# ghostop14/gr-clenabled

Measured on AMD Instinct MI355X. Metric: MSamples/sec (complex-float) through clFFT 4096 fwd + window + shift, higher is better.
Workload: dtype f32; 1 GPU; BASELINE configs[1]: forward clFFT 4096-pt complex, blackman window + fftshift, 16384 frames/step/GPU device-resident (1 GiB in+out); fft_size=4096, parallelism=replica-per-gpu x1

## Files before the change

### gr-clenabled_amd/csrc/fft.hip

```cpp
#include <cmath>
#include <cstdlib>
#include <vector>

#include "common.h"
#include "fft_core.hpp"
#include "fft_mr.h"

using namespace fftc;
#ifndef MI355_FFT_WPE
#define MI355_FFT_WPE 3
#endif

namespace {

typedef float f2v __attribute__((ext_vector_type(2)));

template <int N, bool REAL, class G>
__device__ __forceinline__ void load_group(c32 (&v)[16], const void *__restrict__ in, int grp, int tid, int nframes, int in_xor)
{
    using P = Plan<N>;
    constexpr int TH = G::TH, PTS = G::PTS, F = G::F, R0 = P::radix(0), B0 = N / R0;
    const int frames_left = nframes - grp * F;
    if constexpr (N <= 64) {
        (void)in_xor;
#pragma unroll
        for (int k = 0; k < 16; k++) {
            const unsigned e = (unsigned)(tid + TH * k);
            const bool ok = (int)(e / N) < frames_left;
            if constexpr (REAL) {
                const float x = __builtin_nontemporal_load((const float *)in + (size_t)grp * PTS + (ok ? e : 0u));
                v[k] = mk(ok ? x : 0.f, 0.f);
            } else {
                const f2v x = __builtin_nontemporal_load((const f2v *)in + (size_t)grp * PTS + (ok ? e : 0u));
                v[k] = ok ? mk(x.x, x.y) : mk(0.f, 0.f);
            }
        }
        return;
    }
#pragma unroll
    for (int q = 0; q < 16 / R0; q++) {
        const int g = tid + TH * q, fr = g / B0;
        const bool ok = (F == 1) || fr < frames_left;
        const unsigned off = (unsigned)((ok ? fr * N : 0) + (g % B0));
#pragma unroll
        for (int r = 0; r < R0; r++) {
            const unsigned e = off + (unsigned)((r * B0) ^ in_xor);
            if constexpr (REAL) {
                const float x = __builtin_nontemporal_load((const float *)in + (size_t)grp * PTS + e);
                v[q * R0 + r] = mk(ok ? x : 0.f, 0.f);
            } else {
                const f2v x = __builtin_nontemporal_load((const f2v *)in + (size_t)grp * PTS + e);
                v[q * R0 + r] = ok ? mk(x.x, x.y) : mk(0.f, 0.f);
            }
        }
    }
}

template <int N, int SIGN, bool REAL, int PF, class G>
__global__ __launch_bounds__(G::TH, (N <= 4096 ? (PF == 2 ? 2 : MI355_FFT_WPE) : 1)) void k_fft(const void *__restrict__ in, c32 *__restrict__ out,
                                                                 const float *__restrict__ window,
                                                                 const c32 *__restrict__ twtab, int nframes, int ngroups,
                                                                 int shift)
{
    using P = Plan<N>;
    constexpr int TH = G::TH, PTS = G::PTS, F = G::F, NP = P::NP;
    constexpr bool SMALL = N <= 64;
    constexpr int PAD = (N / P::radix(0)) > 1 ? (N / P::radix(0)) : 1;
    constexpr int LDS_SLOTS = SMALL ? PTS + (PTS / N) * PAD : (NP > 1 ? PTS : 1);
    __shared__ c32 lds[LDS_SLOTS];
    const int tid0 = threadIdx.x;
    const int in_xor = (SIGN > 0 && shift) ? (N >> 1) : 0;
    const int out_xor = (SIGN < 0 && shift) ? (N >> 1) : 0;

    TwRegs<N> tw;
    load_twiddles<N, false, G>(tw, tid0, twtab);
    constexpr int R0 = P::radix(0), B0 = N / R0;
    float win[16];
    if constexpr (SMALL) {
        win[0] = window[tid0 % N];
    } else {
#pragma unroll
        for (int q = 0; q < 16 / R0; q++) {
            const int j = (tid0 + TH * q) % B0;
#pragma unroll
            for (int r = 0; r < R0; r++) win[q * R0 + r] = window[j + ((r * B0) ^ in_xor)];
        }
    }

    auto body = [&](c32 (&cur)[16], int grp, int tid) {
        const int frames_left = nframes - grp * F;
        c32 v[16];
        if constexpr (SMALL) {
            const float wv = win[0];
            const int pos = (tid % N) ^ in_xor, fr0 = tid / N;
#pragma unroll
            for (int k = 0; k < 16; k++) {
                const int fr = fr0 + k * (TH / N);
                lds[fr * (N + PAD) + pos] = scale(cur[k], wv);
            }
            __syncthreads();
#pragma unroll
            for (int q = 0; q < 16 / R0; q++) {
                const int g = tid + TH * q, base = (g / B0) * (N + PAD) + (g % B0);
#pragma unroll
                for (int r = 0; r < R0; r++) v[q * R0 + r] = lds[base + r * B0];
            }
            __syncthreads();
        } else {
#pragma unroll
            for (int s = 0; s < 16; s++) v[s] = scale(cur[s], win[s]);
        }
        transform_regs<N, SIGN, false, G>(v, tw, lds, tid);
        if constexpr (SMALL) {
            constexpr int RL = P::radix(NP - 1), BL = N / RL;
            if constexpr (NP > 1) __syncthreads();
#pragma unroll
            for (int q = 0; q < 16 / RL; q++) {
                const int g = tid + TH * q, base = (g / BL) * (N + PAD) + (g % BL);
#pragma unroll
                for (int s = 0; s < RL; s++) lds[base + ((orev<RL>(s) * BL) ^ out_xor)] = v[q * RL + s];
            }
            __syncthreads();
            f2v *__restrict__ out_g = (f2v *)out + (size_t)grp * PTS;
            const int pos = tid % N, fr0 = tid / N;
#pragma unroll
            for (int k = 0; k < 16; k++) {
                const int fr = fr0 + k * (TH / N);
                if (fr < frames_left) {
                    const c32 z = lds[fr * (N + PAD) + pos];
                    f2v o;
                    o.x = z.x;
                    o.y = z.y;
                    __builtin_nontemporal_store(o, out_g + tid + TH * k);
                }
            }
        } else {
            constexpr int RL = P::radix(NP - 1), BL = N / RL;
            f2v *__restrict__ out_g = (f2v *)out + (size_t)grp * PTS;
#pragma unroll
            for (int q = 0; q < 16 / RL; q++) {
                const int g = tid + TH * q, fr = g / BL;
                const unsigned off = (unsigned)(fr * N + (g % BL));
                if ((F == 1) || fr < frames_left) {
#pragma unroll
                    for (int s = 0; s < RL; s++) {
                        f2v o;
                        o.x = v[q * RL + s].x;
                        o.y = v[q * RL + s].y;
                        __builtin_nontemporal_store(o, out_g + off + (unsigned)((orev<RL>(s) * BL) ^ out_xor));
                    }
                }
            }
        }
        if constexpr (NP > 1 || SMALL) __syncthreads();
    };
    const int stride = gridDim.x;
    if constexpr (PF == 2) {
        c32 b0[16], b1[16], b2[16];
        int grp = blockIdx.x;
        if (grp < ngroups) load_group<N, REAL, G>(b0, in, grp, tid0, nframes, in_xor);
        if (grp + stride < ngroups) load_group<N, REAL, G>(b1, in, grp + stride, tid0, nframes, in_xor);
#define MI355_FFT_STEP(CUR, FREE)                                                                   \
        {                                                                                           \
            if (grp >= ngroups) break;                                                              \
            int tid = tid0;                                                                         \
            asm volatile("" : "+v"(tid));                                                           \
            if (grp + 2 * stride < ngroups) load_group<N, REAL, G>(FREE, in, grp + 2 * stride, tid, nframes, in_xor); \
            __builtin_amdgcn_sched_barrier(0);                                                      \
            body(CUR, grp, tid);                                                                    \
            grp += stride;                                                                          \
        }
        for (;;) {
            MI355_FFT_STEP(b0, b2)
            MI355_FFT_STEP(b1, b0)
            MI355_FFT_STEP(b2, b1)
        }
#undef MI355_FFT_STEP
    } else {
        c32 cur[16];
        if ((int)blockIdx.x < ngroups) load_group<N, REAL, G>(cur, in, blockIdx.x, tid0, nframes, in_xor);
        for (int grp = blockIdx.x; grp < ngroups; grp += stride) {
            int tid = tid0;
            asm volatile("" : "+v"(tid));
            c32 nxt[16];
            if constexpr (PF == 1) {
                const int gnext = grp + stride;
                if (gnext < ngroups) load_group<N, REAL, G>(nxt, in, gnext, tid, nframes, in_xor);
                __builtin_amdgcn_sched_barrier(0);
            } else if (grp != (int)blockIdx.x) {
                load_group<N, REAL, G>(cur, in, grp, tid, nframes, in_xor);
            }
            body(cur, grp, tid);
            if constexpr (PF == 1) {
#pragma unroll
                for (int s = 0; s < 16; s++) cur[s] = nxt[s];
            }
        }
    }
}

typedef float f4v __attribute__((ext_vector_type(4)));
__host__ __device__ constexpr float cos128(int m)
{
    constexpr float t[128] = {1.0f, 0.99879545f, 0.99518472f, 0.989176512f, 0.980785251f, 0.970031261f, 0.956940353f, 0.941544056f, 0.923879504f, 0.903989315f, 0.881921291f, 0.857728601f, 0.831469595f, 0.803207517f, 0.773010433f, 0.740951121f, 0.707106769f, 0.671558976f, 0.634393275f, 0.59569931f, 0.555570245f, 0.514102757f, 0.471396744f, 0.427555084f, 0.382683426f, 0.336889863f, 0.290284663f, 0.242980182f, 0.195090324f, 0.146730468f, 0.0980171412f, 0.0490676761f, 0.0f, -0.0490676761f, -0.0980171412f, -0.146730468f, -0.195090324f, -0.242980182f, -0.290284663f, -0.336889863f, -0.382683426f, -0.427555084f, -0.471396744f, -0.514102757f, -0.555570245f, -0.59569931f, -0.634393275f, -0.671558976f, -0.707106769f, -0.740951121f, -0.773010433f, -0.803207517f, -0.831469595f, -0.857728601f, -0.881921291f, -0.903989315f, -0.923879504f, -0.941544056f, -0.956940353f, -0.970031261f, -0.980785251f, -0.989176512f, -0.99518472f, -0.99879545f, -1.0f, -0.99879545f, -0.99518472f, -0.989176512f, -0.980785251f, -0.970031261f, -0.956940353f, -0.941544056f, -0.923879504f, -0.903989315f, -0.881921291f, -0.857728601f, -0.831469595f, -0.803207517f, -0.773010433f, -0.740951121f, -0.707106769f, -0.671558976f, -0.634393275f, -0.59569931f, -0.555570245f, -0.514102757f, -0.471396744f, -0.427555084f, -0.382683426f, -0.336889863f, -0.290284663f, -0.242980182f, -0.195090324f, -0.146730468f, -0.0980171412f, -0.0490676761f, 0.0f, 0.0490676761f, 0.0980171412f, 0.146730468f, 0.195090324f, 0.242980182f, 0.290284663f, 0.336889863f, 0.382683426f, 0.427555084f, 0.471396744f, 0.514102757f, 0.555570245f, 0.59569931f, 0.634393275f, 0.671558976f, 0.707106769f, 0.740951121f, 0.773010433f, 0.803207517f, 0.831469595f, 0.857728601f, 0.881921291f, 0.903989315f, 0.923879504f, 0.941544056f, 0.956940353f, 0.970031261f, 0.980785251f, 0.989176512f, 0.99518472f, 0.99879545f};
    return t[m & 127];
}
__host__ __device__ constexpr float circ_cos(int m, int circ) { return cos128(m * (128 / circ)); }
__host__ __device__ constexpr float circ_sin(int m, int circ) { return cos128(m * (128 / circ) - 32); }
static_assert(circ_cos(0, 128) == 1.0f && circ_cos(32, 128) == 0.0f && circ_cos(16, 128) == 0.707106781f && circ_sin(32, 128) == 1.0f &&
                  circ_sin(8, 64) == 0.707106781f && circ_cos(16, 32) == -1.0f, "twiddle table");

template <int SIGN, bool REAL>
__global__ __launch_bounds__(512, 2) void k_fft_32k(const void *__restrict__ in, c32 *__restrict__ out, const float *__restrict__ window,
                                                    const c32 *__restrict__ twN, int nframes, int shift)
{
    constexpr int N = 32768, NS = 4096, S = 8, H = 4, BL = 256;
    using G = Geo<NS>;
    __shared__ c32 sm[4 * NS];
    const int set = threadIdx.x >> 8, tid0 = threadIdx.x & 255;
    c32 *lds = sm + set * 2 * NS;
    const int in_xor = (SIGN > 0 && shift) ? 8 : 0;
    const int m_xor = (SIGN < 0 && shift) ? (S / 2) : 0;

#ifndef PFR32K
#define PFR32K 0
#endif
    constexpr int PFW = REAL ? 2 : 4, PFR = REAL ? 2 * PFR32K : PFR32K;
    f4v pf[PFR > 0 ? PFR : 1][PFW];
    auto fetch = [&](int frame, int j, int tid, f4v (&t)[PFW]) {
        const unsigned n = (unsigned)(tid + (((8 * set + j) ^ in_xor) * BL));
        const f4v *p = (const f4v *)in + (size_t)frame * (REAL ? N / 4 : N / 2) + (size_t)n * PFW;
#pragma unroll
        for (int k = 0; k < PFW; k++) t[k] = p[k];
    };
    if ((int)blockIdx.x < nframes) {
#pragma unroll
        for (int j = 0; j < PFR; j++) fetch(blockIdx.x, j, tid0, pf[j]);
    }
    for (int frame = blockIdx.x; frame < nframes; frame += gridDim.x) {
        int tid = tid0;
        asm volatile("" : "+v"(tid));
        c32 v[H][16];
        auto load_frame = [&](auto set_tag) {
            constexpr int SET = decltype(set_tag)::value, OTHER = 1 - SET;
#pragma unroll
            for (int j = 0; j < 8; j++) {
                const int r = 8 * SET + j;
                const unsigned n = (unsigned)(tid + ((r ^ in_xor) * BL));
                const f4v wa = *((const f4v *)window + (size_t)n * 2), wb = *((const f4v *)window + (size_t)n * 2 + 1);
                const float w[8] = {wa.x, wa.y, wa.z, wa.w, wb.x, wb.y, wb.z, wb.w};
                f4v t[PFW];
                if (j < PFR) {
#pragma unroll
                    for (int k = 0; k < PFW; k++) t[k] = pf[j][k];
                } else {
                    fetch(frame, j, tid, t);
                }
                c32 x[S];
                if constexpr (REAL) {
#pragma unroll
// ... 470 lines not shown
        for (int i = 0; i < 32; i++) {
            const int e = tid + TH * i, col = e & 15, row = e >> 4;
            c32 x = pf[i];
            if constexpr (!PASS_B) {
                const float w = window[(size_t)(row ^ row_xor) * ld + c0 + col];
                x = mk(x.x * w, x.y * w);
            }
            tile_lds[col * CS + row] = x;
        }
        __syncthreads();
        c32 va[16], vb[16];
        constexpr int R0 = PL::radix(0), B0 = NR / R0;
#pragma unroll
        for (int q = 0; q < 16 / R0; q++) {
            const int g = tid + TH * q, fr = g / B0, j = g % B0;
#pragma unroll
            for (int r = 0; r < R0; r++) {
                va[q * R0 + r] = tile_lds[fr * CS + j + r * B0];
                vb[q * R0 + r] = tile_lds[(fr + 8) * CS + j + r * B0];
            }
        }
        __syncthreads();
        if (item + gridDim.x < nitems) fetch(item + gridDim.x, pf, tid);
        transform_regs2<NR, SIGN, REV, G>(va, vb, tw, tile_lds, tile_lds + 8 * NR, tid);
        constexpr int NP = PL::NP, RL = PL::radix(NP - 1), BL = NR / RL;
        if constexpr (!PASS_B) {
            static_assert(RL == 16, "reversed plan: the last pass is radix 16");
            const int fr = tid / BL, j = tid % BL;
#pragma unroll
            for (int h = 0; h < 2; h++) {
                const int n2 = c0 + fr + 8 * h;
                const c32 base = twN[(int)(((long long)n2 * j) & nmask)], g1 = twN[(int)(((long long)n2 * BL) & nmask)];
                const c32 g2 = cmul(g1, g1), g4 = cmul(g2, g2), g8 = cmul(g4, g4);
                c32 gp[16];
                gp[0] = base;
                gp[1] = cmul(base, g1);
                gp[2] = cmul(base, g2);
                gp[3] = cmul(gp[2], g1);
                gp[4] = cmul(base, g4);
                gp[5] = cmul(gp[4], g1);
                gp[6] = cmul(gp[4], g2);
                gp[7] = cmul(gp[6], g1);
#pragma unroll
                for (int m = 0; m < 8; m++) gp[8 + m] = cmul(gp[m], g8);
                f2v *__restrict__ o = (f2v *)out + (size_t)frame * frame_elems + (size_t)n2 * NR + j;
#pragma unroll
                for (int t = 0; t < 16; t++) {
                    const c32 z = cmul(h ? vb[t] : va[t], gp[orev<16>(t)]);
                    f2v zz;
                    zz.x = z.x;
                    zz.y = z.y;
                    o[orev<16>(t) * BL] = zz;
                }
            }
            __syncthreads();
        } else {
            __syncthreads();
#pragma unroll
            for (int q = 0; q < 16 / RL; q++) {
                const int g = tid + TH * q, fr = g / BL, j = g % BL;
#pragma unroll
                for (int t = 0; t < RL; t++) {
                    tile_lds[fr * CS + j + orev<RL>(t) * BL] = va[q * RL + t];
                    tile_lds[(fr + 8) * CS + j + orev<RL>(t) * BL] = vb[q * RL + t];
                }
            }
            __syncthreads();
#pragma unroll
            for (int i = 0; i < 32; i++) {
                const int e = tid + TH * i, col = e & 15, row = e >> 4;
                const c32 z = tile_lds[col * CS + row];
                f2v zz;
                zz.x = z.x;
                zz.y = z.y;
                __builtin_nontemporal_store(zz, (f2v *)out + (size_t)frame * frame_elems + (size_t)(row ^ row_xor) * ld + c0 + col);
            }
            __syncthreads();
        }
    }
}

template <int N, class G>
int launch_g(mi355_ctx *ctx, int sign, const void *in, void *out, const float *window, const void *tw, int nframes, int shift,
             int real_in, hipStream_t st)
{
    constexpr int F = G::F, TH = G::TH, WAVES = TH / 64;
    int ngroups = (nframes + F - 1) / F;
    int cus = ctx->num_cus > 0 ? ctx->num_cus : 256;
    int pf = getenv("MI355_FFT_PREFETCH") ? atoi(getenv("MI355_FFT_PREFETCH")) : -1;
    const bool persistent2 = N <= 4096 && WAVES == 4 && ngroups >= cus * 2 * 8;
    if (pf < 0) pf = persistent2 ? 1 : 0;
    int grid = (N <= 4096) ? mi355_balanced_grid(ctx, ngroups, 32 / WAVES, 64 / WAVES, 0.015) : mi355_balanced_grid(ctx, ngroups, 1, 1);
    if (pf == 1 && persistent2) grid = cus * 2;
    if (const char *e = getenv("MI355_FFT_WG_PER_CU")) {
        if (atoi(e) > 0) grid = ngroups < cus * atoi(e) ? ngroups : cus * atoi(e);
    }
#define LAUNCH_FFT(SG, RL)                                                                                              \
    do {                                                                                                                     \
        if (pf == 2)                                                                                                         \
            hipLaunchKernelGGL((k_fft<N, SG, RL, 2, G>), dim3(grid), dim3(TH), 0, st, in, (c32 *)out, window, (const c32 *)tw, \
                               nframes, ngroups, shift);                                                                     \
        else if (pf == 1)                                                                                                    \
            hipLaunchKernelGGL((k_fft<N, SG, RL, 1, G>), dim3(grid), dim3(TH), 0, st, in, (c32 *)out, window, (const c32 *)tw, \
                               nframes, ngroups, shift);                                                                     \
        else                                                                                                                 \
            hipLaunchKernelGGL((k_fft<N, SG, RL, 0, G>), dim3(grid), dim3(TH), 0, st, in, (c32 *)out, window,                \
                               (const c32 *)tw, nframes, ngroups, shift);                                                    \
    } while (0)
    if (sign < 0) { if (real_in) LAUNCH_FFT(-1, true); else LAUNCH_FFT(-1, false); }
    else          { if (real_in) LAUNCH_FFT(1, true);  else LAUNCH_FFT(1, false); }
#undef LAUNCH_FFT
    MI355_HIP(hipGetLastError());
    return MI355_OK;
}

template <int N>
int launch_n(mi355_ctx *ctx, int sign, const void *in, void *out, const float *window, const void *tw, int nframes, int shift,
             int real_in, hipStream_t st)
{
    if constexpr (N >= 16 && N <= 1024) {
        static const bool wave = getenv("MI355_FFT_WAVE_GEO") ? atoi(getenv("MI355_FFT_WAVE_GEO")) != 0 : false;
        if (wave) return launch_g<N, GeoW<N>>(ctx, sign, in, out, window, tw, nframes, shift, real_in, st);
    }
    if constexpr (N == 32768) return launch_s<N>(ctx, sign, in, out, window, tw, nframes, shift, real_in, st);
    else if constexpr (N == 8192 || N == 16384) {
        static const bool whole = getenv("MI355_FFT_WHOLE_FRAME") ? atoi(getenv("MI355_FFT_WHOLE_FRAME")) != 0 : false;
        if (!whole) return launch_s<N>(ctx, sign, in, out, window, tw, nframes, shift, real_in, st);
    }
    if constexpr (N != 32768) return launch_g<N, Geo<N>>(ctx, sign, in, out, window, tw, nframes, shift, real_in, st);
}

int launch_fft(mi355_ctx *ctx, int n, int sign, const void *in, void *out, const float *window, const void *tw, int nframes,
               int shift, int real_in, hipStream_t st)
{
    switch (n) {
#define CASE_N(NN) case NN: return launch_n<NN>(ctx, sign, in, out, window, tw, nframes, shift, real_in, st)
        CASE_N(2); CASE_N(4); CASE_N(8); CASE_N(16); CASE_N(32); CASE_N(64); CASE_N(128); CASE_N(256); CASE_N(512);
        CASE_N(1024); CASE_N(2048); CASE_N(4096); CASE_N(8192); CASE_N(16384); CASE_N(32768);
#undef CASE_N
    }
    mi355_set_error("fft size %d unsupported (power of two, 2..32768)", n);
    return MI355_ERR_UNSUPPORTED;
}

}

struct mi355_fft {
    mi355_ctx *ctx;
    int n, sign, dtype, nstreams, shift;
    float *d_window;
    void *d_tw;
    HostPipe pipe;
    MrPlan mr;
    MrTilePlan mrt;
    int m = 0;
    void *d_pre = nullptr, *d_post = nullptr, *d_bspec = nullptr;
    void *d_twm_f = nullptr, *d_twm_i = nullptr;
    float *d_ones = nullptr;
    mi355_fft *sub_f = nullptr, *sub_i = nullptr;
    void *d_wa = nullptr, *d_wb = nullptr;
    size_t cap_frames = 0;
    bool two_kernel = false;
    int tile_n1 = 0, tile_n2 = 0;
    std::mutex ws_lock;
    hipEvent_t ws_done = nullptr;
    bool ws_used = false;
};

namespace {

__global__ __launch_bounds__(256) void k_blu_pre(const void *__restrict__ in, c32 *__restrict__ A, const c32 *__restrict__ pre,
                                                 const int *__restrict__ src, int N, int M, long long total, int real_in)
{
    for (long long e = (long long)blockIdx.x * 256 + threadIdx.x; e < total; e += (long long)gridDim.x * 256) {
        const long long f = e / M;
        const int m = (int)(e - f * M);
        c32 v = mk(0.f, 0.f);
        if (m < N) {
            const int i = src[m];
            const c32 x = real_in ? mk(((const float *)in)[f * N + i], 0.f) : ((const c32 *)in)[f * N + i];
            v = cmul(x, pre[m]);
        }
        A[e] = v;
    }
}

__global__ __launch_bounds__(256) void k_blu_mul(c32 *__restrict__ B, const c32 *__restrict__ bspec, int M, long long total)
{
    for (long long e = (long long)blockIdx.x * 256 + threadIdx.x; e < total; e += (long long)gridDim.x * 256)
        B[e] = cmul(B[e], bspec[e & (M - 1)]);
}

__global__ __launch_bounds__(256) void k_blu_post(const c32 *__restrict__ A, c32 *__restrict__ out, const c32 *__restrict__ post,
                                                  int N, int M, long long total, int lo)
{
    for (long long e = (long long)blockIdx.x * 256 + threadIdx.x; e < total; e += (long long)gridDim.x * 256) {
        const long long f = e / N;
        const int p = (int)(e - f * N);
        const int k = lo ? (p < N - lo ? p + lo : p - (N - lo)) : p;
        out[e] = cmul(A[f * M + k], post[k]);
    }
}

template <int M, bool REAL>
__global__ __launch_bounds__(Geo<M>::TH, Geo<M>::WPE) void k_chirpz(const void *__restrict__ in, c32 *__restrict__ out,
                                                                   const c32 *__restrict__ pre, const int *__restrict__ src,
                                                                   const c32 *__restrict__ post, const c32 *__restrict__ bspec,
                                                                   const c32 *__restrict__ tw_fwd, const c32 *__restrict__ tw_inv,
                                                                   int N, int nframes, int ngroups, int lo)
{
    using G = Geo<M>;
    using PF = Plan<M, false>;
    using PI = Plan<M, true>;
    constexpr int TH = G::TH, F = G::F, NP = PF::NP;
    constexpr int RL = PF::radix(NP - 1), BL = M / RL;
    static_assert(PI::radix(0) == RL, "inverse plan must start with the forward plan's last radix");
    extern __shared__ __attribute__((aligned(16))) c32 chirp_lds[];
    c32 *lds = chirp_lds;
    const int tid0 = threadIdx.x;
    constexpr bool SHARE = (PF::L % 4) == 0;
    TwRegs<M> twf, twi;
    load_twiddles<M, false, G>(twf, tid0, tw_fwd);
    if constexpr (!SHARE) load_twiddles<M, true, G>(twi, tid0, tw_inv);
    c32 Breg[16];
#pragma unroll
    for (int q = 0; q < 16 / RL; q++) {
        const int j = (tid0 + TH * q) % BL;
#pragma unroll
        for (int t = 0; t < RL; t++) Breg[q * RL + t] = bspec[j + orev<RL>(t) * BL];
    }
    for (int grp = blockIdx.x; grp < ngroups; grp += gridDim.x) {
        int tid = tid0;
        asm volatile("" : "+v"(tid));
        const int frames_left = nframes - grp * F;
        const size_t fbase = (size_t)grp * F;
        c32 v[16];
        constexpr int R0 = PF::radix(0), B0 = M / R0;
#pragma unroll
        for (int q = 0; q < 16 / R0; q++) {
            const int g = tid + TH * q, fr = g / B0, j = g % B0;
#pragma unroll
            for (int r = 0; r < R0; r++) {
                const int m = j + r * B0;
                const bool ok = m < N && fr < frames_left;
                c32 x = mk(0.f, 0.f);
                if (ok) {
                    const int i = src[m];
                    if constexpr (REAL) x = mk(((const float *)in)[(fbase + fr) * N + i], 0.f);
// ... 255 lines not shown
            }
            {
                const long long total = (long long)nf * 1048576;
                long long blocks = (total + 255) / 256;
                if (blocks > (long long)cus * 16) blocks = (long long)cus * 16;
                const int mx = (h->sign < 0 && h->shift) ? S3 / 2 : 0;
#define COMB2G(SS) do { if (h->sign < 0) COMB2(SS, -1, 1, (const c32 *)h->d_wa, dst, (const c32 *)h->d_tw, total, 1048576, (long long)N, 1048576LL, 0LL, 0LL, 1, N - 1, mx); \
                        else             COMB2(SS, 1, 1, (const c32 *)h->d_wa, dst, (const c32 *)h->d_tw, total, 1048576, (long long)N, 1048576LL, 0LL, 0LL, 1, N - 1, mx); } while (0)
                if (S3 == 2) COMB2G(2); else if (S3 == 4) COMB2G(4); else if (S3 == 8) COMB2G(8); else COMB2G(16);
#undef COMB2G
            }
            MI355_HIP(hipGetLastError());
            continue;
        }
        if (three_pass) {
            const int S2 = S / 16;
            {
                const long long total = (long long)nf * 4096;
                long long blocks = (total + 255) / 256;
                if (blocks > (long long)cus * 16 / S2 + 1) blocks = (long long)cus * 16 / S2 + 1;
                if (h->sign < 0) COMB2(16, -1, S2, (const c32 *)h->d_wa, (c32 *)h->d_wb, (const c32 *)h->d_tw, total, 4096, (long long)N, (long long)S2 * 4096, 4096LL, 65536LL, S2, N - 1, 0);
                else             COMB2(16, 1, S2, (const c32 *)h->d_wa, (c32 *)h->d_wb, (const c32 *)h->d_tw, total, 4096, (long long)N, (long long)S2 * 4096, 4096LL, 65536LL, S2, N - 1, 0);
            }
            {
                const long long total = (long long)nf * 65536;
                long long blocks = (total + 255) / 256;
                if (blocks > (long long)cus * 16) blocks = (long long)cus * 16;
                const int mx = (h->sign < 0 && h->shift) ? S2 / 2 : 0;
#define COMB2F(SS) do { if (h->sign < 0) COMB2(SS, -1, 1, (const c32 *)h->d_wb, dst, (const c32 *)h->d_tw, total, 65536, (long long)N, 65536LL, 0LL, 0LL, 1, N - 1, mx); \
                        else             COMB2(SS, 1, 1, (const c32 *)h->d_wb, dst, (const c32 *)h->d_tw, total, 65536, (long long)N, 65536LL, 0LL, 0LL, 1, N - 1, mx); } while (0)
                if (S2 == 2) COMB2F(2); else if (S2 == 4) COMB2F(4); else if (S2 == 8) COMB2F(8); else COMB2F(16);
#undef COMB2F
            }
            MI355_HIP(hipGetLastError());
            continue;
        }
#undef COMB2
        const long long total = (long long)nf * 4096;
        long long blocks = (total + 255) / 256;
        if (blocks > (long long)cus * 16) blocks = (long long)cus * 16;
#define COMB(SS, SG) hipLaunchKernelGGL((k_fft_combine<SS, SG>), dim3((unsigned)blocks), dim3(256), 0, st, (const c32 *)h->d_wa, dst, (const c32 *)h->d_tw, total, m_xor)
        if (S == 8) { if (h->sign < 0) COMB(8, -1); else COMB(8, 1); }
        else        { if (h->sign < 0) COMB(16, -1); else COMB(16, 1); }
#undef COMB
        MI355_HIP(hipGetLastError());
    }
    return ws_release(h, st);
}

int launch_mr_tile(mi355_fft *h, const void *in, void *out, int nframes, hipStream_t st)
{
    const size_t N = (size_t)h->n;
    size_t chunk = ((size_t)256 << 20) / (N * 8);
    if (chunk < 1) chunk = 1;
    if (chunk > (size_t)nframes) chunk = (size_t)nframes;
    std::lock_guard<std::mutex> ws_guard(h->ws_lock);
    {
        const int rc = ws_acquire(h, st, chunk > h->cap_frames);
        if (rc) return rc;
    }
    if (chunk > h->cap_frames) {
        MI355_HIP(hipStreamSynchronize(st));
        if (h->d_wa) (void)hipFree(h->d_wa);
        h->d_wa = nullptr; h->cap_frames = 0;
        MI355_HIP(hipMalloc(&h->d_wa, chunk * N * 8));
        h->cap_frames = chunk;
    }
    const size_t isz = h->dtype == MI355_DTYPE_FLOAT ? 4 : 8;
    for (size_t f0 = 0; f0 < (size_t)nframes; f0 += chunk) {
        const int nf = (int)((size_t)nframes - f0 < chunk ? (size_t)nframes - f0 : chunk);
        const int rc = mi355_fft_mr_tile_launch(h->mrt, h->ctx, h->sign, (const char *)in + f0 * N * isz, h->d_wa, (char *)out + f0 * N * 8, h->d_window, nf,
                                                h->shift, h->dtype == MI355_DTYPE_FLOAT, st);
        if (rc) return rc;
    }
    return ws_release(h, st);
}

int launch_handle(mi355_fft *h, const void *in, void *out, int nvec, hipStream_t st)
{
    if (h->mrt.n) return launch_mr_tile(h, in, out, nvec, st);
    if (h->mr.n) return mi355_fft_mr_launch(h->mr, h->ctx, h->sign, in, out, h->d_window, nvec, h->shift, h->dtype == MI355_DTYPE_FLOAT, st);
    if (h->m) return launch_bluestein(h, in, out, nvec, st);
    if (h->n > 32768 || (h->n == 32768 && h->two_kernel)) return launch_big(h, in, out, nvec, st);
    return launch_fft(h->ctx, h->n, h->sign, in, out, h->d_window, h->d_tw, nvec, h->shift, h->dtype == MI355_DTYPE_FLOAT, st);
}

void host_fft_pow2(std::vector<double> &re, std::vector<double> &im, int sign)
{
    const int n = (int)re.size();
    for (int i = 1, j = 0; i < n; i++) {
        int bit = n >> 1;
        for (; j & bit; bit >>= 1) j ^= bit;
        j ^= bit;
        if (i < j) { std::swap(re[i], re[j]); std::swap(im[i], im[j]); }
    }
    std::vector<double> cr(n / 2 > 0 ? n / 2 : 1), ci(n / 2 > 0 ? n / 2 : 1);
    for (int k = 0; k < n / 2; k++) {
        const double a = sign * 2.0 * M_PI * (double)k / (double)n;
        cr[k] = cos(a);
        ci[k] = sin(a);
    }
    for (int len = 2; len <= n; len <<= 1) {
        const int step = n / len;
        for (int i = 0; i < n; i += len)
            for (int k = 0; k < len / 2; k++) {
                const double wr = cr[(size_t)k * step], wi = ci[(size_t)k * step];
                const int p = i + k, q = p + len / 2;
                const double tr = re[q] * wr - im[q] * wi, ti = re[q] * wi + im[q] * wr;
                re[q] = re[p] - tr; im[q] = im[p] - ti;
                re[p] += tr; im[p] += ti;
            }
    }
}

int upload(mi355_ctx *ctx, void **d, const void *src, size_t bytes)
{
    if (hipMalloc(d, bytes) != hipSuccess) return MI355_ERR_NOMEM;
    if (mi355_upload(ctx, *d, src, bytes) != hipSuccess) return MI355_ERR_HIP;
    return MI355_OK;
}

std::vector<float> twiddle_table(int n, int sign)
{
    std::vector<float> tw;
    tw.reserve(2 * (size_t)n + 8192);
    for (int k = 0; k < n; k++) {
        const double a = sign * 2.0 * M_PI * (double)k / (double)n;
        tw.push_back((float)cos(a));
        tw.push_back((float)sin(a));
    }
    if (n > 4096)
        for (int k = 0; k < 4096; k++) {
            const double a = sign * 2.0 * M_PI * (double)k / 4096.0;
            tw.push_back((float)cos(a));
            tw.push_back((float)sin(a));
        }
    return tw;
}

int setup_bluestein(mi355_fft *h, const float *window)
{
    const int N = h->n;
    int M = 256;
    while (M < 2 * N - 1) M <<= 1;
    h->m = M;
    std::vector<double> ar(N), ai(N);
    for (int n = 0; n < N; n++) {
        const long long q = ((long long)n * n) % (2LL * N);
        const double ang = h->sign * M_PI * (double)q / (double)N;
        ar[n] = cos(ang); ai[n] = sin(ang);
    }
    const int half = N / 2;
    const bool rshift = h->sign > 0 && h->shift;
    std::vector<float> pre(2 * (size_t)N), post(2 * (size_t)N);
    std::vector<int> src(N);
    for (int m = 0; m < N; m++) {
        const int i = rshift ? (m >= N - half ? m - (N - half) : m + half) : m;
        src[m] = i;
        const double w = window ? (double)window[i] : 1.0;
        pre[2 * m] = (float)(w * ar[m]); pre[2 * m + 1] = (float)(w * ai[m]);
        post[2 * m] = (float)ar[m]; post[2 * m + 1] = (float)ai[m];
    }
    std::vector<double> br(M, 0.0), bi(M, 0.0);
    for (int n = 0; n < N; n++) {
        br[n] = ar[n]; bi[n] = -ai[n];
        if (n) { br[M - n] = ar[n]; bi[M - n] = -ai[n]; }
    }
    host_fft_pow2(br, bi, -1);
    std::vector<float> bs(2 * (size_t)M);
    for (int k = 0; k < M; k++) { bs[2 * k] = (float)(br[k] / M); bs[2 * k + 1] = (float)(bi[k] / M); }
    std::vector<char> post_blob((size_t)N * 8 + (size_t)N * 4);
    memcpy(post_blob.data(), post.data(), (size_t)N * 8);
    memcpy(post_blob.data() + (size_t)N * 8, src.data(), (size_t)N * 4);
    int rc;
    if ((rc = upload(h->ctx, &h->d_pre, pre.data(), pre.size() * 4))) return rc;
    if ((rc = upload(h->ctx, &h->d_post, post_blob.data(), post_blob.size()))) return rc;
    if ((rc = upload(h->ctx, &h->d_bspec, bs.data(), bs.size() * 4))) return rc;
    if (M > 32768) {
        if ((rc = mi355_fft_create(h->ctx, M, MI355_FFT_FORWARD, nullptr, 0, MI355_DTYPE_COMPLEX, 1, 0, &h->sub_f))) return rc;
        return mi355_fft_create(h->ctx, M, MI355_FFT_BACKWARD, nullptr, 0, MI355_DTYPE_COMPLEX, 1, 0, &h->sub_i);
    }
    std::vector<float> tf = twiddle_table(M, -1), ti = twiddle_table(M, 1), ones(M, 1.0f);
    if ((rc = upload(h->ctx, &h->d_twm_f, tf.data(), tf.size() * 4))) return rc;
    if ((rc = upload(h->ctx, &h->d_twm_i, ti.data(), ti.size() * 4))) return rc;
    if ((rc = upload(h->ctx, (void **)&h->d_ones, ones.data(), ones.size() * 4))) return rc;
    return MI355_OK;
}

}

extern "C" int mi355_fft_create(mi355_ctx *ctx, int fft_size, int direction, const float *window, int window_len, int dtype,
                                int num_streams, int shift, mi355_fft **out)
{
    MI355_REQUIRE(ctx && out, "NULL argument");
    *out = nullptr;
    const bool pow2 = fft_size >= 2 && (fft_size & (fft_size - 1)) == 0;
    if (fft_size < 2 || (pow2 && fft_size > 16777216) || (!pow2 && fft_size > 8388608)) {
        mi355_set_error("fft size %d unsupported (powers of two 2..16777216, any other size 3..8388608)", fft_size);
        return fft_size < 2 ? MI355_ERR_INVALID_ARG : MI355_ERR_UNSUPPORTED;
    }
    MI355_REQUIRE(window_len == 0 || window_len == fft_size, "window not the same length as fft_size");
    MI355_REQUIRE(window_len == 0 || window != nullptr, "window is NULL");
    MI355_REQUIRE(dtype == MI355_DTYPE_COMPLEX || dtype == MI355_DTYPE_FLOAT, "clFFT dtype must be complex or float");
    MI355_REQUIRE(num_streams >= 1, "num_streams must be >= 1");
    mi355_fft *h = new (std::nothrow) mi355_fft();
    if (!h) return MI355_ERR_NOMEM;
    h->ctx = ctx; h->n = fft_size;
    h->sign = (direction == MI355_FFT_FORWARD) ? -1 : 1;
    h->dtype = dtype; h->nstreams = num_streams; h->shift = shift ? 1 : 0;
    h->d_window = nullptr; h->d_tw = nullptr;
    auto fail = [&](int rc) { mi355_fft_destroy(h); return rc; };
    if (hipSetDevice(ctx->device) != hipSuccess) return fail(MI355_ERR_HIP);
    std::vector<float> tw(2 * (size_t)fft_size);
    for (int k = 0; k < fft_size; k++) {
        double a = h->sign * 2.0 * M_PI * (double)k / (double)fft_size;
        tw[2 * k] = (float)cos(a);
        tw[2 * k + 1] = (float)sin(a);
    }
    if (fft_size > 4096) {
        for (int k = 0; k < 4096; k++) {
            double a = h->sign * 2.0 * M_PI * (double)k / 4096.0;
            tw.push_back((float)cos(a));
            tw.push_back((float)sin(a));
        }
    }
    if (pow2 && fft_size >= 65536 && fft_size <= 1048576 && !getenv("MI355_FFT_NO_TILE")) {
        int lg = 0;
        while ((1 << lg) < fft_size) lg++;
        h->tile_n1 = lg == 17 ? 256 : 1 << ((lg + 1) / 2);
        if (const char *e = getenv("MI355_FFT_TILE_N1")) {
            const int v = atoi(e);
            if ((v == 256 || v == 512 || v == 1024) && fft_size / v >= 256 && fft_size / v <= 1024) h->tile_n1 = v;
        }
        h->tile_n2 = fft_size / h->tile_n1;
        for (int nr : {h->tile_n1, h->tile_n2})
            for (int k = 0; k < nr; k++) {
                double a = h->sign * 2.0 * M_PI * (double)k / (double)nr;
                tw.push_back((float)cos(a));
                tw.push_back((float)sin(a));
            }
    }
    if (hipMalloc(&h->d_tw, tw.size() * sizeof(float)) != hipSuccess) return fail(MI355_ERR_NOMEM);
    if (mi355_upload(ctx, h->d_tw, tw.data(), tw.size() * sizeof(float)) != hipSuccess) return fail(MI355_ERR_HIP);
    {
        std::vector<float> w(fft_size, 1.0f);
        if (window_len) memcpy(w.data(), window, sizeof(float) * (size_t)fft_size);
        h->two_kernel = pow2 && (fft_size > 32768 || (fft_size == 32768 && getenv("MI355_FFT_32768_TWO_KERNELS") != nullptr));
        if (h->two_kernel && !h->tile_n1) {
            const int S = fft_size / 4096;
            std::vector<float> p((size_t)fft_size);
            for (int sq = 0; sq < S / 4; sq++)
                for (int n = 0; n < 4096; n++)
                    for (int j = 0; j < 4; j++) p[((size_t)sq * 4096 + n) * 4 + j] = w[(size_t)n * S + 4 * sq + j];
            w.swap(p);
        }
        if (hipMalloc((void **)&h->d_window, sizeof(float) * (size_t)fft_size) != hipSuccess) return fail(MI355_ERR_NOMEM);
        if (mi355_upload(ctx, h->d_window, w.data(), sizeof(float) * (size_t)fft_size) != hipSuccess)
            return fail(MI355_ERR_HIP);
    }
    int rc = h->pipe.init(ctx);
    if (rc) return fail(rc);
    if (!pow2) {
        std::vector<float> mtw;
        if (!getenv("MI355_FFT_NO_MR") && mi355_fft_mr_plan(fft_size, h->sign, 0, &h->mr, &mtw)) {
            auto put = [&](MrPlan &pl, const std::vector<float> &t) {
                if (hipMalloc(&pl.d_tw, t.size() * sizeof(float)) != hipSuccess) return (int)MI355_ERR_NOMEM;
                return mi355_upload(ctx, pl.d_tw, t.data(), t.size() * sizeof(float)) != hipSuccess ? (int)MI355_ERR_HIP : (int)MI355_OK;
            };
            int known = mi355_fft_mr_cached_variant(fft_size);
            if (known < 0 && !getenv("MI355_FFT_MR_TIMED_VARIANT")) known = (fft_size == 96 || fft_size == 100 || fft_size == 2400) ? 1 : 0;
            if (const char *e = getenv("MI355_FFT_MR_VARIANT")) known = atoi(e) != 0 ? 1 : 0;
            MrPlan alt;
            std::vector<float> atw;
            const bool have_alt = mi355_fft_mr_plan(fft_size, h->sign, 1, &alt, &atw) && (alt.npass != h->mr.npass || alt.per_thread != h->mr.per_thread);
            if (known == 1 && have_alt) {
                h->mr = alt;
                mtw.swap(atw);
            }
            if ((rc = put(h->mr, mtw))) return fail(rc);
            float ms0 = -1.f, ms1 = -1.f;
            if ((rc = mi355_fft_mr_tune(&h->mr, ctx, h->sign, h->d_window, &ms0))) return fail(rc);
            if (known < 0 && have_alt && ms0 > 0.f && getenv("MI355_FFT_MR_TIMED_VARIANT")) {
                if ((rc = put(alt, atw))) { if (alt.d_tw) (void)hipFree(alt.d_tw); return fail(rc); }
                rc = mi355_fft_mr_tune(&alt, ctx, h->sign, h->d_window, &ms1);
                if (rc) { (void)hipFree(alt.d_tw); return fail(rc); }
                if (ms1 > 0.f && ms1 < ms0 * 0.90f) {
                    (void)hipFree(h->mr.d_tw);
                    h->mr = alt;
                } else {
                    (void)hipFree(alt.d_tw);
                }
            }
            if (ms0 > 0.f) {
                mi355_fft_mr_remember(h->mr);
                mi355_log(ctx, MI355_LOG_INFO, "clFFT %d points (mixed radix): %d passes, %d threads x %d frame(s) per workgroup measured fastest", fft_size,
                          h->mr.npass, h->mr.threads, h->mr.frames);
            }
        } else {
            h->mr.n = 0;
            std::vector<float> twa, twb;
            if (!getenv("MI355_FFT_NO_MR") && mi355_fft_mr_tile_plan(fft_size, h->sign, &h->mrt, &twa, &twb)) {
                h->mrt.a.d_tw = h->mrt.b.d_tw = nullptr;
                if (hipMalloc(&h->mrt.a.d_tw, twa.size() * sizeof(float) + 8) != hipSuccess) return fail(MI355_ERR_NOMEM);
                if (hipMalloc(&h->mrt.b.d_tw, twb.size() * sizeof(float) + 8) != hipSuccess) return fail(MI355_ERR_NOMEM);
                if (!twa.empty() && mi355_upload(ctx, h->mrt.a.d_tw, twa.data(), twa.size() * sizeof(float)) != hipSuccess) return fail(MI355_ERR_HIP);
                if (!twb.empty() && mi355_upload(ctx, h->mrt.b.d_tw, twb.data(), twb.size() * sizeof(float)) != hipSuccess) return fail(MI355_ERR_HIP);
                h->mrt.d_twn = h->d_tw;
            } else {
                h->mrt.n = 0;
                rc = setup_bluestein(h, window_len ? window : nullptr);
                if (rc) return fail(rc);
            }
        }
    }
    mi355_log(ctx, MI355_LOG_INFO, "clFFT: %d points, %s, %s input, %d stream(s), shift %d, window %s: %s", fft_size,
              h->sign < 0 ? "forward" : "reverse", dtype == MI355_DTYPE_COMPLEX ? "complex" : "float", num_streams, h->shift,
              window_len ? "given" : "none",
              h->mr.n ? "mixed radix, one pass" : h->mrt.n ? "mixed radix, two passes over sixteen-column tiles" : !pow2 ? "chirp-z over a power-of-two transform" : h->tile_n1 ? "two passes over 16-column tiles" : h->two_kernel ? "multi-pass" : "one pass");
    *out = h;
    return MI355_OK;
}

extern "C" int mi355_fft_plan_text(int fft_size, char *buf, int buf_len)
{
    MI355_REQUIRE(buf && buf_len > 0, "NULL argument");
    const bool pow2 = fft_size >= 2 && (fft_size & (fft_size - 1)) == 0;
    if (fft_size < 2 || (pow2 && fft_size > 16777216) || (!pow2 && fft_size > 8388608)) {
        snprintf(buf, (size_t)buf_len, "unsupported (powers of two 2..16777216, any other size 3..8388608)");
        return MI355_ERR_UNSUPPORTED;
    }
    if (pow2) {
        if (fft_size <= 32768) snprintf(buf, (size_t)buf_len, "one pass");
        else if (fft_size <= 1048576) {
            int lg = 0;
            while ((1 << lg) < fft_size) lg++;
            const int n1 = lg == 17 ? 256 : 1 << ((lg + 1) / 2);
            snprintf(buf, (size_t)buf_len, "two tile passes %d x %d", n1, fft_size / n1);
        } else snprintf(buf, (size_t)buf_len, "four passes");
        return MI355_OK;
    }
    MrPlan mp;
    std::vector<float> tw;
    if (mi355_fft_mr_plan(fft_size, -1, 0, &mp, &tw)) {
        int at = snprintf(buf, (size_t)buf_len, "mixed radix ");
        for (int p = 0; p < mp.npass && at < buf_len; p++) at += snprintf(buf + at, (size_t)(buf_len - at), p ? " x %d" : "%d", mp.pass[p].radix);
        return MI355_OK;
    }
    MrTilePlan tp;
    std::vector<float> twb;
    if (mi355_fft_mr_tile_plan(fft_size, -1, &tp, &tw, &twb)) {
        snprintf(buf, (size_t)buf_len, "mixed radix, two passes %d x %d", tp.n1, tp.n2);
        return MI355_OK;
    }
    int m = 256;
    while (m < 2 * fft_size - 1) m <<= 1;
    snprintf(buf, (size_t)buf_len, "chirp-z, m = %d%s", m, m <= 16384 ? " (fused)" : "");
    return MI355_OK;
}

const MrPlan *mi355_fft_mr_plan_of(const mi355_fft *h, int *sign)
{
    if (!h || !h->mr.n) return nullptr;
    if (sign) *sign = h->sign;
    return &h->mr;
}

extern "C" int mi355_fft_destroy(mi355_fft *h)
{
    if (!h) return MI355_OK;
    (void)hipSetDevice(h->ctx->device);
    h->pipe.release();
    if (h->d_window) (void)hipFree(h->d_window);
    if (h->d_tw) (void)hipFree(h->d_tw);
    if (h->mr.d_tw) (void)hipFree(h->mr.d_tw);
    if (h->mrt.a.d_tw) (void)hipFree(h->mrt.a.d_tw);
    if (h->mrt.b.d_tw) (void)hipFree(h->mrt.b.d_tw);
    for (void *p : {h->d_pre, h->d_post, h->d_bspec, h->d_twm_f, h->d_twm_i, (void *)h->d_ones, h->d_wa, h->d_wb})
        if (p) (void)hipFree(p);
    if (h->ws_done) (void)hipEventDestroy(h->ws_done);
    if (h->sub_f) (void)mi355_fft_destroy(h->sub_f);
    if (h->sub_i) (void)mi355_fft_destroy(h->sub_i);
    delete h;
    return MI355_OK;
}

extern "C" int mi355_fft_work_dev(mi355_fft *h, int nvec, const void *in, void *out, void *stream)
{
    MI355_REQUIRE(h != nullptr, "handle is NULL");
    if (nvec <= 0) return MI355_OK;
    MI355_REQUIRE(in && out, "NULL buffer");
    MI355_REQUIRE((reinterpret_cast<uintptr_t>(in) & 7u) == 0 && (reinterpret_cast<uintptr_t>(out) & 7u) == 0,
                  "device buffers must be 8-byte aligned");
    MI355_REQUIRE(h->m != 0 || h->n <= 4096 || (reinterpret_cast<uintptr_t>(in) & 15u) == 0,
                  "device input of an 8192/16384-point transform must be 16-byte aligned");
    MI355_HIP(hipSetDevice(h->ctx->device));
    return launch_handle(h, in, out, nvec, mi355_pick_stream(h->ctx, stream));
}

extern "C" int mi355_fft_work(mi355_fft *h, int nvec, const void *const *in_streams, void *const *out_streams)
{
    MI355_REQUIRE(h != nullptr, "handle is NULL");
    if (nvec <= 0) return MI355_OK;
    MI355_REQUIRE(in_streams && out_streams, "NULL stream arrays");
    std::lock_guard<std::mutex> g(h->ctx->lock);
    MI355_HIP(hipSetDevice(h->ctx->device));
    const size_t isz = mi355_dtype_size(h->dtype), in_frame = isz * (size_t)h->n, out_frame = 8 * (size_t)h->n;
    size_t chunk_frames = mi355_chunk_bytes((size_t)nvec * out_frame) / out_frame;
    if (chunk_frames < 1) chunk_frames = 1;
    size_t first = (size_t)nvec < chunk_frames ? (size_t)nvec : chunk_frames;
    size_t inb = first * in_frame;
    const int nslots = first * out_frame >= ((size_t)32 << 20) ? 2 : HostPipe::kSlots;
    int rc = h->pipe.ensure(1, &inb, first * out_frame, nslots);
    if (rc) return rc;
    HostPipe &p = h->pipe;
    if ((size_t)nvec <= chunk_frames && mi355_direct_ok((size_t)nvec * out_frame)) {
        hipStream_t st = h->ctx->stream[0];
        for (int s_i = 0; s_i < h->nstreams; s_i++) {
            MI355_REQUIRE(in_streams[s_i] && out_streams[s_i], "NULL stream buffer");
            mi355_copy(p.h_in[0][0], in_streams[s_i], (size_t)nvec * in_frame);
            rc = launch_handle(h, p.h_in[0][0], p.h_out[0], nvec, st);
            if (rc) return rc;
            MI355_HIP(mi355_direct_sync(st));
            mi355_copy(out_streams[s_i], p.h_out[0], (size_t)nvec * out_frame);
        }
        return MI355_OK;
    }
    size_t nchunks = ((size_t)nvec + chunk_frames - 1) / chunk_frames;
    char *pend_dst[HostPipe::kSlots] = {};
    size_t pend_bytes[HostPipe::kSlots] = {};
    size_t seq = 0;
    const bool one_stream = h->m || h->mrt.n || h->n > 32768 || (h->n == 32768 && h->two_kernel);
    for (int s_i = 0; s_i < h->nstreams; s_i++) {
        MI355_REQUIRE(in_streams[s_i] && out_streams[s_i], "NULL stream buffer");
        const char *pin = (const char *)in_streams[s_i];
        char *pout = (char *)out_streams[s_i];
        for (size_t ci = 0; ci < nchunks; ci++, seq++) {
            int s = (int)(seq % nslots);
            hipStream_t st = h->ctx->stream[one_stream ? 0 : (s & 1)];
            size_t f0 = ci * chunk_frames;
            size_t nf = (size_t)nvec - f0 < chunk_frames ? (size_t)nvec - f0 : chunk_frames;
            if (pend_bytes[s]) MI355_HIP(hipEventSynchronize(p.done[s]));
            mi355_copy2(pend_dst[s], p.h_out[s], pend_bytes[s], p.h_in[s][0], pin + f0 * in_frame, nf * in_frame);
            pend_bytes[s] = 0;
            MI355_HIP(hipMemcpyAsync(p.d_in[s][0], p.h_in[s][0], nf * in_frame, hipMemcpyHostToDevice, st));
            rc = launch_handle(h, p.d_in[s][0], p.d_out[s], (int)nf, st);
            if (rc) return rc;
            MI355_HIP(hipMemcpyAsync(p.h_out[s], p.d_out[s], nf * out_frame, hipMemcpyDeviceToHost, st));
            MI355_HIP(hipEventRecord(p.done[s], st));
            pend_dst[s] = pout + f0 * out_frame;
            pend_bytes[s] = nf * out_frame;
        }
    }
    for (int q = 0; q < nslots; q++) {
        int s = (int)((seq + q) % nslots);
        if (pend_bytes[s]) {
            MI355_HIP(hipEventSynchronize(p.done[s]));
// ... 7 lines not shown
```

Baseline: 387,900 MSamples/s.

## Add per-XCD atomic work hand-out to persistent FFT kernel

Replaces the static grid-stride group assignment in the persistent one-group-prefetch FFT kernel with dynamic scheduling. Each workgroup draws its next frame group from one of eight atomic counters, one per XCD, so groups stay XCD-local while load imbalance between workgroups is absorbed. Per-stream counter buffers are allocated and reset by the last finishing block. The cost is an atomic plus a __syncthreads per group and extra host-side stream bookkeeping under a mutex.

```diff
diff --git a/gr-clenabled_amd/csrc/fft.hip b/gr-clenabled_amd/csrc/fft.hip
--- a/gr-clenabled_amd/csrc/fft.hip
+++ b/gr-clenabled_amd/csrc/fft.hip
@@ -56,11 +56,11 @@
     }
 }
 
-template <int N, int SIGN, bool REAL, int PF, class G>
+template <int N, int SIGN, bool REAL, int PF, class G, bool DYN = false>
 __global__ __launch_bounds__(G::TH, (N <= 4096 ? (PF == 2 ? 2 : MI355_FFT_WPE) : 1)) void k_fft(const void *__restrict__ in, c32 *__restrict__ out,
                                                                  const float *__restrict__ window,
                                                                  const c32 *__restrict__ twtab, int nframes, int ngroups,
-                                                                 int shift)
+                                                                 int shift, unsigned *__restrict__ ctr = nullptr)
 {
     using P = Plan<N>;
     constexpr int TH = G::TH, PTS = G::PTS, F = G::F, NP = P::NP;
@@ -176,6 +176,37 @@
             MI355_FFT_STEP(b2, b1)
         }
 #undef MI355_FFT_STEP
+    } else if constexpr (DYN) {
+        static_assert(PF == 1, "the hand-out is built on the one-group register prefetch");
+        __shared__ int handout;
+        const int G8 = (int)gridDim.x / 8, xcd = (int)blockIdx.x % 8;
+        auto draw = [&]() { return xcd + 8 * ((int)atomicAdd(ctr + 32 * xcd, 1u) + G8); };
+        if (tid0 == 0) handout = draw();
+        __syncthreads();
+        int grp = blockIdx.x, gnext = handout;
+        c32 cur[16];
+        if (grp < ngroups) load_group<N, REAL, G>(cur, in, grp, tid0, nframes, in_xor);
+        while (grp < ngroups) {
+            int tid = tid0;
+            asm volatile("" : "+v"(tid));
+            c32 nxt[16];
+            if (gnext < ngroups) load_group<N, REAL, G>(nxt, in, gnext, tid, nframes, in_xor);
+            int drawn = ngroups;
+            if (tid0 == 0 && gnext < ngroups) drawn = draw();
+            __builtin_amdgcn_sched_barrier(0);
+            body(cur, grp, tid);
+            if (tid0 == 0) handout = drawn;
+            __syncthreads();
+            grp = gnext;
+            gnext = handout;
+#pragma unroll
+            for (int s = 0; s < 16; s++) cur[s] = nxt[s];
+        }
+        __syncthreads();
+        if (tid0 == 0 && atomicAdd(ctr + 256, 1u) == gridDim.x - 1) {
+            for (int x = 0; x < 8; x++) atomicExch(ctr + 32 * x, 0u);
+            atomicExch(ctr + 256, 0u);
+        }
     } else {
         c32 cur[16];
         if ((int)blockIdx.x < ngroups) load_group<N, REAL, G>(cur, in, blockIdx.x, tid0, nframes, in_xor);
@@ -812,7 +843,7 @@
 
 template <int N, class G>
 int launch_g(mi355_ctx *ctx, int sign, const void *in, void *out, const float *window, const void *tw, int nframes, int shift,
-             int real_in, hipStream_t st)
+             int real_in, hipStream_t st, unsigned *ctr)
 {
     constexpr int F = G::F, TH = G::TH, WAVES = TH / 64;
     int ngroups = (nframes + F - 1) / F;
@@ -825,17 +856,25 @@
     if (const char *e = getenv("MI355_FFT_WG_PER_CU")) {
         if (atoi(e) > 0) grid = ngroups < cus * atoi(e) ? ngroups : cus * atoi(e);
     }
+    const char *ho = getenv("MI355_FFT_HANDOUT");
+    const bool dyn = N >= 256 && ctr != nullptr && pf == 1 && persistent2 && grid % 8 == 0 && (ho == nullptr || atoi(ho) != 0);
 #define LAUNCH_FFT(SG, RL)                                                                                              \
     do {                                                                                                                     \
+        if constexpr (N >= 256)                                                                                              \
+            if (dyn) {                                                                                                       \
+                hipLaunchKernelGGL((k_fft<N, SG, RL, 1, G, true>), dim3(grid), dim3(TH), 0, st, in, (c32 *)out, window,      \
+                                   (const c32 *)tw, nframes, ngroups, shift, ctr);                                           \
+                break;                                                                                                       \
+            }                                                                                                                \
         if (pf == 2)                                                                                                         \
             hipLaunchKernelGGL((k_fft<N, SG, RL, 2, G>), dim3(grid), dim3(TH), 0, st, in, (c32 *)out, window, (const c32 *)tw, \
-                               nframes, ngroups, shift);                                                                     \
+                               nframes, ngroups, shift, nullptr);                                                            \
         else if (pf == 1)                                                                                                    \
             hipLaunchKernelGGL((k_fft<N, SG, RL, 1, G>), dim3(grid), dim3(TH), 0, st, in, (c32 *)out, window, (const c32 *)tw, \
-                               nframes, ngroups, shift);                                                                     \
+                               nframes, ngroups, shift, nullptr);                                                            \
         else                                                                                                                 \
             hipLaunchKernelGGL((k_fft<N, SG, RL, 0, G>), dim3(grid), dim3(TH), 0, st, in, (c32 *)out, window,                \
-                               (const c32 *)tw, nframes, ngroups, shift);                                                    \
+                               (const c32 *)tw, nframes, ngroups, shift, nullptr);                                           \
     } while (0)
     if (sign < 0) { if (real_in) LAUNCH_FFT(-1, true); else LAUNCH_FFT(-1, false); }
     else          { if (real_in) LAUNCH_FFT(1, true);  else LAUNCH_FFT(1, false); }
@@ -846,25 +885,25 @@
 
 template <int N>
 int launch_n(mi355_ctx *ctx, int sign, const void *in, void *out, const float *window, const void *tw, int nframes, int shift,
-             int real_in, hipStream_t st)
+             int real_in, hipStream_t st, unsigned *ctr)
 {
     if constexpr (N >= 16 && N <= 1024) {
         static const bool wave = getenv("MI355_FFT_WAVE_GEO") ? atoi(getenv("MI355_FFT_WAVE_GEO")) != 0 : false;
-        if (wave) return launch_g<N, GeoW<N>>(ctx, sign, in, out, window, tw, nframes, shift, real_in, st);
+        if (wave) return launch_g<N, GeoW<N>>(ctx, sign, in, out, window, tw, nframes, shift, real_in, st, nullptr);
     }
     if constexpr (N == 32768) return launch_s<N>(ctx, sign, in, out, window, tw, nframes, shift, real_in, st);
     else if constexpr (N == 8192 || N == 16384) {
         static const bool whole = getenv("MI355_FFT_WHOLE_FRAME") ? atoi(getenv("MI355_FFT_WHOLE_FRAME")) != 0 : false;
         if (!whole) return launch_s<N>(ctx, sign, in, out, window, tw, nframes, shift, real_in, st);
     }
-    if constexpr (N != 32768) return launch_g<N, Geo<N>>(ctx, sign, in, out, window, tw, nframes, shift, real_in, st);
+    if constexpr (N != 32768) return launch_g<N, Geo<N>>(ctx, sign, in, out, window, tw, nframes, shift, real_in, st, ctr);
 }
 
 int launch_fft(mi355_ctx *ctx, int n, int sign, const void *in, void *out, const float *window, const void *tw, int nframes,
-               int shift, int real_in, hipStream_t st)
+               int shift, int real_in, hipStream_t st, unsigned *ctr = nullptr)
 {
     switch (n) {
-#define CASE_N(NN) case NN: return launch_n<NN>(ctx, sign, in, out, window, tw, nframes, shift, real_in, st)
+#define CASE_N(NN) case NN: return launch_n<NN>(ctx, sign, in, out, window, tw, nframes, shift, real_in, st, ctr)
         CASE_N(2); CASE_N(4); CASE_N(8); CASE_N(16); CASE_N(32); CASE_N(64); CASE_N(128); CASE_N(256); CASE_N(512);
         CASE_N(1024); CASE_N(2048); CASE_N(4096); CASE_N(8192); CASE_N(16384); CASE_N(32768);
 #undef CASE_N
@@ -894,6 +933,11 @@
     int tile_n1 = 0, tile_n2 = 0;
     std::mutex ws_lock;
     hipEvent_t ws_done = nullptr;
+    static constexpr int kHandoutStreams = 16, kHandoutWords = 512;
+    unsigned *d_handout = nullptr;
+    hipStream_t handout_st[kHandoutStreams] = {};
+    int handout_n = 0;
+    std::mutex handout_lock;
     bool ws_used = false;
 };
 
@@ -1315,7 +1359,15 @@
     if (h->mr.n) return mi355_fft_mr_launch(h->mr, h->ctx, h->sign, in, out, h->d_window, nvec, h->shift, h->dtype == MI355_DTYPE_FLOAT, st);
     if (h->m) return launch_bluestein(h, in, out, nvec, st);
     if (h->n > 32768 || (h->n == 32768 && h->two_kernel)) return launch_big(h, in, out, nvec, st);
-    return launch_fft(h->ctx, h->n, h->sign, in, out, h->d_window, h->d_tw, nvec, h->shift, h->dtype == MI355_DTYPE_FLOAT, st);
+    unsigned *ctr = nullptr;
+    if (h->d_handout) {
+        std::lock_guard<std::mutex> g(h->handout_lock);
+        int i = 0;
+        while (i < h->handout_n && h->handout_st[i] != st) i++;
+        if (i == h->handout_n && i < mi355_fft::kHandoutStreams) h->handout_st[h->handout_n++] = st;
+        if (i < h->handout_n) ctr = h->d_handout + (size_t)i * mi355_fft::kHandoutWords;
+    }
+    return launch_fft(h->ctx, h->n, h->sign, in, out, h->d_window, h->d_tw, nvec, h->shift, h->dtype == MI355_DTYPE_FLOAT, st, ctr);
 }
 
 void host_fft_pow2(std::vector<double> &re, std::vector<double> &im, int sign)
@@ -1475,6 +1527,11 @@
     }
     if (hipMalloc(&h->d_tw, tw.size() * sizeof(float)) != hipSuccess) return fail(MI355_ERR_NOMEM);
     if (mi355_upload(ctx, h->d_tw, tw.data(), tw.size() * sizeof(float)) != hipSuccess) return fail(MI355_ERR_HIP);
+    if (pow2 && fft_size >= 256 && fft_size <= 4096) {
+        const std::vector<unsigned> zero((size_t)mi355_fft::kHandoutStreams * mi355_fft::kHandoutWords, 0u);
+        if (hipMalloc(&h->d_handout, zero.size() * sizeof(unsigned)) != hipSuccess) return fail(MI355_ERR_NOMEM);
+        if (mi355_upload(ctx, h->d_handout, zero.data(), zero.size() * sizeof(unsigned)) != hipSuccess) return fail(MI355_ERR_HIP);
+    }
     {
         std::vector<float> w(fft_size, 1.0f);
         if (window_len) memcpy(w.data(), window, sizeof(float) * (size_t)fft_size);
@@ -1605,6 +1662,7 @@
     h->pipe.release();
     if (h->d_window) (void)hipFree(h->d_window);
     if (h->d_tw) (void)hipFree(h->d_tw);
+    if (h->d_handout) (void)hipFree(h->d_handout);
     if (h->mr.d_tw) (void)hipFree(h->mr.d_tw);
     if (h->mrt.a.d_tw) (void)hipFree(h->mrt.a.d_tw);
     if (h->mrt.b.d_tw) (void)hipFree(h->mrt.b.d_tw);
```

After: 388,300 MSamples/s, median of 6. No clear change (+0.1%).
